# Mattdl/CLsurvey

Measured on AMD Instinct MI355X. Metric: images/sec (train+importance pass), EWC small_VGG9 Tiny-ImageNet task batch, higher is better.
Workload: dtype f32 (bf16x6 split operands on the conv fwd/bwd-data matrix products, fp32 accumulate); 1 GPU; EWC small_VGG9_cl_128_128, Tiny-ImageNet shapes (3x64x64, 20 classes), batch 200: train step + Fisher step (BASELINE configs[1]); batch=200, parallelism=1 GPU

## Files before the change

### clsurvey_amd/_lib.py

```python
import ctypes as C
import os

_HERE = os.path.dirname(os.path.abspath(__file__))
LIB_PATH = os.path.join(_HERE, "libclhip.so")

_p = C.c_void_p
_i = C.c_int
_f = C.c_float
_z = C.c_size_t
_l = C.c_long


class HatParam(C.Structure):
    _fields_ = [("theta", _p), ("grad", _p), ("buf", _p), ("mask_back", _p), ("n", _z), ("is_emb", _i), ("reserved", _i)]


class HatGateJob(C.Structure):
    _fields_ = [("emb_row", _p), ("gate", _p), ("mask_pre", _p), ("n", _i), ("reserved", _i)]


class HatLayer(C.Structure):
    _fields_ = [("w", _p), ("gate_in", _p), ("out", _p), ("K", _z), ("C", _z), ("R", _z)]


class HatWgradJob(C.Structure):
    _fields_ = [("g", _p), ("w", _p), ("gate_in", _p), ("dgate_in", _p), ("K", _i), ("C", _i), ("R", _i), ("reserved", _i)]


class HatEmbJob(C.Structure):
    _fields_ = [("dgate", _p), ("gate", _p), ("mask_pre", _p), ("demb", _p), ("n", _i), ("rows", _i), ("t", _i), ("reserved", _i)]


class PathnetLayer(C.Structure):
    _fields_ = [("w_off", _l), ("b_off", _l), ("pw_off", _l), ("pb_off", _l), ("mod_stride", _l), ("c_out", _i), ("c_in", _i),
                ("R", _i), ("n_out", _i), ("n_in", _i), ("Kp", _i), ("Cp", _i), ("M", _i), ("path", _i * 8),
                ("trainable", C.c_ulonglong)]


class IcarlClass(C.Structure):
    _fields_ = [("row_begin", _i), ("row_end", _i), ("k", _i), ("out_off", _i)]


class ReduceJob(C.Structure):
    _fields_ = [("slabs", _p), ("dw", _p), ("db", _p), ("K", _i), ("C", _i), ("splits", _i), ("taps", _i)]


class LayerDesc(C.Structure):
    _fields_ = [("type", _i), ("cin", _i), ("cout", _i), ("relu", _i), ("pool", _i),
                ("w_off", _l), ("b_off", _l), ("ksize", _i), ("stride", _i), ("pad", _i), ("pool_k", _i), ("pool_s", _i),
                ("bn", _i), ("bn_w_off", _l), ("bn_b_off", _l), ("has_drop", _i)]


SIGNATURES = {
    "clhip_version": (_i, []),
    "clhip_arch": (C.c_char_p, []),
    "clhip_conv3x3_fwd": (_i, [_p, _p, _p, _p, _i, _i, _i, _i, _i, _i, _p]),
    "clhip_conv3x3_relu_pool_fwd": (_i, [_p, _p, _p, _p, _p, _i, _i, _i, _i, _i, _p]),
    "clhip_conv3x3_bwd_weight_unpool": (_i, [_p, _p, _p, _p, _p, _i, _i, _i, _i, _i, _p, _z, _p]),
    "clhip_conv3x3_bwd_data": (_i, [_p, _p, _p, _p, _i, _i, _i, _i, _i, _p]),
    "clhip_conv3x3_bwd_data_unpool": (_i, [_p, _p, _p, _p, _p, _i, _i, _i, _i, _i, _p]),
    "clhip_conv3x3_bwd_weight_ws": (_z, [_i, _i, _i, _i, _i]),
    "clhip_conv3x3_bwd_weight": (_i, [_p, _p, _p, _p, _i, _i, _i, _i, _i, _p, _z, _p]),
    "clhip_conv3x3_bwd_weight_slabs": (_i, [_p, _p, _p, _i, _i, _i, _i, _i, _p, _z, C.POINTER(_i), _p]),
    "clhip_conv3x3_bwd_weight_reduce": (_i, [_p, _p, _p, _i, _i, _i, _p]),
    "clhip_conv3x3_wino_ws": (_z, [_i, _i]),
    "clhip_conv3x3_wino_fwd": (_i, [_p, _p, _p, _p, _p, _i, _i, _i, _i, _i, _i, _p, _z, _p]),
    "clhip_conv3x3_wino_bwd_data": (_i, [_p, _p, _p, _p, _p, _i, _i, _i, _i, _i, _p, _z, _p]),
    "clhip_conv5x5_bs_ws": (_z, [_i, _i]),
    "clhip_conv5x5_bs_fwd": (_i, [_p, _p, _p, _p, _i, _i, _i, _i, _i, _i, _p, _z, _p]),
    "clhip_conv5x5_bs_bwd_data": (_i, [_p, _p, _p, _p, _i, _i, _i, _i, _i, _p, _z, _p]),
    "clhip_conv3x3_bs_ws": (_z, [_i, _i]),
    "clhip_conv3x3_bs_fwd": (_i, [_p, _p, _p, _p, _p, _i, _i, _i, _i, _i, _i, _p, _z, _p]),
    "clhip_conv3x3_bs_bwd_data": (_i, [_p, _p, _p, _p, _p, _i, _i, _i, _i, _i, _p, _z, _p]),
    "clhip_conv3x3_bs_bwd_data_riders": (_i, [_p, _p, _p, _p, _p, _i, _i, _i, _i, _i, _p, _z, C.POINTER(ReduceJob), _i, _i, _i, _p]),
    "clhip_conv3x3_wino_bwd_weight_ws": (_z, [_i, _i, _i, _i, _i]),
    "clhip_conv3x3_wino_bwd_weight": (_i, [_p, _p, _p, _p, _p, _i, _i, _i, _i, _i, _p, _z, _p]),
    "clhip_conv3x3_wino_bwd_ws": (_z, [_i, _i, _i, _i, _i]),
    "clhip_conv3x3_wino_bwd": (_i, [_p, _p, _p, _p, _p, _p, _p, _p, _i, _i, _i, _i, _i, _p, _z, _p]),
    "clhip_maxpool2_fwd": (_i, [_p, _p, _p, _i, _i, _i, _p]),
    "clhip_maxpool2_bwd": (_i, [_p, _p, _p, _i, _i, _i, _p]),
    "clhip_fc_ws": (_z, [_i, _i, _i]),
    "clhip_fc_fwd": (_i, [_p, _p, _p, _p, _i, _i, _i, _i, _p, _z, _p]),
    "clhip_fc_bwd_data": (_i, [_p, _p, _p, _p, _i, _i, _i, _p, _z, _p]),
    "clhip_fc_bwd_weight": (_i, [_p, _p, _p, _p, _i, _i, _i, _p, _z, _p]),
    "clhip_relu_bwd": (_i, [_p, _p, _p, _z, _p]),
    "clhip_softmax_ce": (_i, [_p, _p, _i, _i, _i, _p, _p, _p, _p]),
    "clhip_mse_zero_sum": (_i, [_p, _z, _p, _p, _p]),
    "clhip_reg_sgd_step": (_i, [_p, _p, _p, _p, _p, _z, _f, _f, _f, _f, _i, _p]),
    "clhip_fisher_accum": (_i, [_p, _p, _z, _f, _p]),
    "clhip_mas_accum": (_i, [_p, _p, _z, _f, _f, _p]),
    "clhip_si_step": (_i, [_p, _p, _p, _p, _p, _p, _z, _f, _f, _f, _f, _i, _p]),
    "clhip_si_consolidate": (_i, [_p, _p, _p, _p, _z, _f, _p]),
    "clhip_maxpool_fwd": (_i, [_p, _p, _p, _i, _i, _i, _i, _i, _p]),
    "clhip_maxpool_bwd": (_i, [_p, _p, _p, _i, _i, _i, _i, _i, _p]),
    "clhip_conv2d_bwd_weight_ws": (_z, [_i] * 9),
    "clhip_conv2d_fwd": (_i, [_p, _p, _p, _p] + [_i] * 10 + [_p]),
    "clhip_conv2d_bwd_data": (_i, [_p, _p, _p, _p] + [_i] * 9 + [_p]),
    "clhip_conv2d_bwd_weight": (_i, [_p, _p, _p, _p] + [_i] * 9 + [_p, _z, _p]),
    "clhip_conv3x3_bs_bwd_weight_ws": (_z, [_i] * 5),
    "clhip_conv3x3_bs_bwd_weight": (_i, [_p] * 5 + [_i] * 5 + [_p, _z, _p]),
    "clhip_conv5x5_bs_bwd_weight_ws": (_z, [_i] * 5),
    "clhip_conv5x5_bs_bwd_weight": (_i, [_p] * 4 + [_i] * 5 + [_p, _z, _p]),
    "clhip_conv2d_s2d_ws": (_z, [_i] * 8),
    "clhip_conv2d_s2d_fwd": (_i, [_p, _p, _p, _p] + [_i] * 9 + [_p, _z, _p]),
    "clhip_conv2d_s2d_bwd_weight": (_i, [_p, _p, _p, _p] + [_i] * 8 + [_p, _z, _p]),
    "clhip_imm_merge": (_i, [_p, _p, _p, _i, _z, _p, _p]),
    "clhip_lwf_loss": (_i, [_p, _p, _p, _p, _i, _i, _i, _i, _f, _f, _i, _p, _p, _p, _p]),
    "clhip_packnet_finetune_mask": (_i, [_p, _z, _i, _p]),
    "clhip_packnet_kth_ws": (_z, []),
    "clhip_packnet_kth_abs": (_i, [_p, _p, _z, _i, _z, _p, _p, _z, _p]),
    "clhip_packnet_prune": (_i, [_p, _p, _z, _i, _p, _p]),
    "clhip_mask_grad_zero": (_i, [_p, _p, _z, _i, _p]),
    "clhip_mask_weight_zero": (_i, [_p, _p, _z, _i, _i, _p]),
    "clhip_packnet_sgd_step": (_i, [_p, _p, _p, _p, _z, _i, _f, _f, _f, _i, _p]),
    "clhip_hat_gate": (_i, [_p, _i, _f, _p, _p]),
    "clhip_hat_scale_weight": (_i, [_p, _p, _p, _z, _z, _z, _p]),
    "clhip_hat_weight_grad": (_i, [_p, _p, _p, _p, _p, _i, _i, _i, _p]),
    "clhip_hat_emb_grad": (_i, [_p, _p, _p, _i, _f, _f, _p, _p]),
    "clhip_hat_reg_sums": (_i, [_p, _p, _i, _p, _p]),
    "clhip_hat_backmask": (_i, [_p, _p, _p, _z, _z, _z, _p]),
    "clhip_hat_sgd_ws": (_z, []),
    "clhip_hat_sgd_step": (_i, [_p, _p, _p, _p, _z, _f, _f, _f, _i, _i, _f, _f, _f, _f, _i, _p, _z, _p]),
    "clhip_clamp": (_i, [_p, _z, _f, _f, _p]),
    "clhip_hat_sgd_multi_ws": (_z, [_i]),
    "clhip_hat_sgd_step_multi": (_i, [_p, _i, _f, _f, _f, _i, _f, _f, _f, _f, _f, _i, _p, _z, _p]),
    "clhip_hat_gates_multi": (_i, [_p, _i, _f, _p, _p]),
    "clhip_hat_scale_weights_multi": (_i, [_p, _i, _p]),
    "clhip_hat_weight_grads_multi": (_i, [_p, _i, _p]),
    "clhip_hat_emb_grads_multi": (_i, [_p, _i, _f, _f, _f, _p, _p]),
    "clhip_pathnet_ws": (_z, [_p, _i]),
    "clhip_pathnet_pack_multi": (_i, [_p, _i, _p, _z, _p, _z, _p]),
    "clhip_pathnet_fold_grads_multi": (_i, [_p, _i, _p, _z, _p, _z, _p, _z, _p]),
    "clhip_pathnet_sgd_step": (_i, [_p, _i, _p, _p, _p, _z, _f, _f, _f, _f, _i, _p, _z, _p]),
    "clhip_softmax_ce_slice": (_i, [_p, _p, _i, _i, _i, _i, _i, _p, _p, _p, _p]),
    "clhip_net_loss_step_slice": (_i, [_p, _p, _p, _p, _p, _i, _i, _i, _i, _p, _p, _p, _p, _p]),
    "clhip_axpy": (_i, [_p, _p, _z, _f, _i, _p]),
    "clhip_gem_gram_ws": (_z, [_i]),
    "clhip_gem_gram": (_i, [_p, _z, C.POINTER(_i), _i, _z, _p, _p, _z, _p]),
    "clhip_gem_project": (_i, [_p, _z, C.POINTER(_i), C.POINTER(_f), _i, _p, _p, _z, _p]),
    "clhip_gem_qp": (_i, [_p, _i, C.c_double, C.c_double, _p, _p, _p]),
# ... 101 lines not shown
```

### clsurvey_amd/build.py

```python
import glob
import os
import subprocess
import sys

HERE = os.path.dirname(os.path.abspath(__file__))
CSRC = os.path.join(HERE, "csrc")
OUT = os.path.join(HERE, "libclhip.so")
SOURCES = ["elementwise.hip", "loss.hip", "pool.hip", "conv3x3.hip", "wino.hip", "bsconv.hip", "bswgrad.hip", "bswgrad5.hip", "conv3x3_wgrad.hip", "conv2d.hip", "convkk.hip", "s2dconv.hip", "bn.hip", "gemm.hip", "fc_chain.hip",
           "packnet.hip", "hat.hip", "pathnet.hip", "gem.hip", "gem_wide.hip", "rehearsal.hip", "joint.hip", "augment.hip", "icarl.hip", "icarl_assemble.hip", "engine.hip"]
FLAGS = ["--offload-arch=gfx950", "-O3", "-std=c++17", "-fPIC", "-fvisibility=hidden", "-Wall", "-Wno-unused-function",
         "-mllvm", "-pragma-unroll-threshold=100000"]


EXTRA_FLAGS = {"wino.hip": ["-fno-slp-vectorize"]}


def _fingerprint(paths, flags):
    import hashlib
    h = hashlib.sha256(" ".join(flags).encode())
    for path in paths:
        with open(path, "rb") as f:
            h.update(f.read())
    return h.hexdigest()


def build(force=False, verbose=True):
    hipcc = os.environ.get("HIPCC", "/opt/rocm/bin/hipcc")
    objs = []
    hdrs = sorted(glob.glob(os.path.join(CSRC, "*.hpp"))) + [os.path.join(HERE, "..", "include", "clhip.h")]
    procs = []
    for src in SOURCES:
        s = os.path.join(CSRC, src)
        o = os.path.join(CSRC, src.replace(".hip", ".o"))
        stamp = o + ".sha256"
        objs.append(o)
        flags = FLAGS + EXTRA_FLAGS.get(src, [])
        want = _fingerprint([s] + hdrs, flags)
        have = open(stamp).read().strip() if os.path.exists(stamp) and os.path.exists(o) else ""
        if force or have != want:
            cmd = [hipcc] + flags + ["-c", s, "-o", o]
            if verbose:
                print(" ".join(cmd), flush=True)
            if os.path.exists(stamp):
                os.remove(stamp)
            procs.append((src, stamp, want, subprocess.Popen(cmd)))
    for src, stamp, want, p in procs:
        if p.wait() != 0:
            raise RuntimeError("hipcc failed on " + src)
        with open(stamp, "w") as f:
            f.write(want + "\n")
    if force or procs or not os.path.exists(OUT):
        cmd = [hipcc, "--offload-arch=gfx950", "-shared", "-fPIC", "-o", OUT] + objs
        if verbose:
            print(" ".join(cmd), flush=True)
        subprocess.check_call(cmd)
    return OUT


TEST_LIB_SRC = os.path.join(HERE, "..", "tests", "csrc", "debug_naive.hip")
TEST_LIB = os.path.join(HERE, "..", "tests", "libclhip_dbg.so")


def build_test_lib(force=False, verbose=True):
    hipcc = os.environ.get("HIPCC", "/opt/rocm/bin/hipcc")
    stamp = TEST_LIB + ".sha256"
    want = _fingerprint([TEST_LIB_SRC, os.path.join(CSRC, "common.hpp"), os.path.join(HERE, "..", "include", "clhip.h")], FLAGS)
    have = open(stamp).read().strip() if os.path.exists(stamp) and os.path.exists(TEST_LIB) else ""
    if force or have != want:
        cmd = [hipcc] + FLAGS + ["-shared", "-o", TEST_LIB, TEST_LIB_SRC]
        if verbose:
            print(" ".join(cmd), flush=True)
        subprocess.check_call(cmd)
        with open(stamp, "w") as f:
            f.write(want + "\n")
    return TEST_LIB


def build_variant(name, src, defines, verbose=True, extra_flags=()):
    hipcc = os.environ.get("HIPCC", "/opt/rocm/bin/hipcc")
    build(verbose=verbose)
    srcs = [src] if isinstance(src, str) else list(src)
    procs = []
    for s in srcs:
        o = os.path.join(CSRC, s.replace(".hip", ".%s.o" % name))
        cmd = [hipcc] + FLAGS + EXTRA_FLAGS.get(s, []) + list(extra_flags) + ["-D" + d for d in defines] + ["-c", os.path.join(CSRC, s), "-o", o]
        if verbose:
            print(" ".join(cmd), flush=True)
        procs.append(subprocess.Popen(cmd))
    for p in procs:
        if p.wait() != 0:
            raise RuntimeError("hipcc failed on variant " + name)
    objs = [os.path.join(CSRC, x.replace(".hip", ".%s.o" % name if x in srcs else ".o")) for x in SOURCES]
    out = os.path.join(HERE, "libclhip_%s.so" % name)
    subprocess.check_call([hipcc, "--offload-arch=gfx950", "-shared", "-fPIC", "-o", out] + objs)
    return out


# ... 4 lines not shown
```

### clsurvey_amd/csrc/common.hpp

```cpp
#pragma once
#include <hip/hip_runtime.h>
#include <stdint.h>
#include <stddef.h>
#include "../../include/clhip.h"

#define CLHIP_LAUNCH_CHECK()                          \
    do {                                              \
        hipError_t e__ = hipGetLastError();           \
        if (e__ != hipSuccess) return (int)e__;       \
    } while (0)

static inline hipStream_t as_stream(void* s) { return reinterpret_cast<hipStream_t>(s); }

static inline bool aligned16(const void* p) { return (reinterpret_cast<uintptr_t>(p) & 15u) == 0; }

static inline bool clhip_conv3x3_dims_ok(int N, int C, int K, int H, int W) {
    if (N <= 0 || C <= 0 || K <= 0 || H <= 0 || W <= 0) return false;
    const long long hw = (long long)H * W;
    if (hw >= (1LL << 23)) return false;
    if (hw * (C + 32LL) >= (1LL << 28) || hw * (K + 32LL) >= (1LL << 28)) return false;
    if ((long long)K * C >= (1LL << 29) / 9) return false;
    return hw * N <= 0x7fffffffLL;
}

// ... 45 lines not shown
    __builtin_amdgcn_raw_buffer_store_b128(q, r, voff, soff, CLHIP_ST_AUX);
}
__device__ __forceinline__ void clhip_buf_store2(float2 v, __amdgpu_buffer_rsrc_t r, int voff, int soff) {
    typedef unsigned int u32x2 __attribute__((ext_vector_type(2)));
    const u32x2 q = {__float_as_uint(v.x), __float_as_uint(v.y)};
    __builtin_amdgcn_raw_buffer_store_b64(q, r, voff, soff, CLHIP_ST_AUX);
}
__device__ __forceinline__ __amdgpu_buffer_rsrc_t clhip_out_rsrc(void* base) {
    return __builtin_amdgcn_make_buffer_rsrc(base, 0, 0x7fffffff, 0x00020000);
}
__device__ __forceinline__ size_t out_img_of(int C, int hw) { return (size_t)C * hw; }

__device__ __forceinline__ float wave_max(float v) {
#pragma unroll
    for (int o = 32; o > 0; o >>= 1) v = fmaxf(v, __shfl_xor(v, o, 64));
    return v;
}
__device__ __forceinline__ float wave_sum(float v) {
#pragma unroll
    for (int o = 32; o > 0; o >>= 1) v += __shfl_xor(v, o, 64);
    return v;
}
__device__ __forceinline__ double wave_sum(double v) {
#pragma unroll
    for (int o = 32; o > 0; o >>= 1) v += __shfl_xor(v, o, 64);
    return v;
}
__device__ __forceinline__ int wave_min(int v) {
#pragma unroll
    for (int o = 32; o > 0; o >>= 1) v = min(v, __shfl_xor(v, o, 64));
    return v;
}

typedef float floatx16 __attribute__((ext_vector_type(16)));
typedef float floatx4 __attribute__((ext_vector_type(4)));

__device__ __forceinline__ int mfma32_row(int r, int lane) { return (r & 3) + 8 * (r >> 2) + 4 * (lane >> 5); }


#define CLHIP_FC_MAX 4
struct clhip_fc_chain {
    int n;
    long w_off[CLHIP_FC_MAX], b_off[CLHIP_FC_MAX];
    int din[CLHIP_FC_MAX], dout[CLHIP_FC_MAX], relu[CLHIP_FC_MAX];
    size_t act_off[CLHIP_FC_MAX], dz_off[CLHIP_FC_MAX];
};
int clhip_internal_fc_chain_ok(const clhip_fc_chain* d);
int clhip_internal_fc_chain_wgrad(const clhip_fc_chain* d, float* grads, const float* x, int N, const float* acts,
                                  const float* dlogits, const float* dz, hipStream_t s);
struct clhip_gemm_args {
    const float* a; const float* b; float* out;
    int M, N, K; long sam, sak, sbk, sbn; int n_tiles, splits, k_per_split;
    const float* bias; const float* mask_src; int relu;
};
int clhip_internal_fc_bwd_data_args(const float* dy, const float* w, const float* relu_src, float* dx, int M, int I, int O,
                                    clhip_gemm_args* args_out);
int clhip_internal_fc_bwd_combo(const clhip_gemm_args* g, int gemm_blocks, const clhip_fc_chain* d, float* grads, const float* x,
                                int N, const float* acts, const float* dlogits, const float* dz, hipStream_t s);

int clhip_internal_fc_tail_ok(const clhip_fc_chain* d);
int clhip_internal_fc_tail(const clhip_fc_chain* d, const float* params, float* acts, int N, const int64_t* labels,
                           int reduction, int col_off, int ncols, float* dlogits, float* fcdz, float* loss_out, double* stats,
                           void* row_scratch, unsigned* counter, int do_loss, int do_bwd, const float* h1_slabs, int live,
                           hipStream_t s);
int clhip_internal_fc_fwd_partial(const float* x, const float* w, int M, int I, int O, void* ws, size_t ws_bytes, int* live,
                                  hipStream_t s);

#define CLHIP_WGRAD_JOBS_MAX 32
struct clhip_wgrad_job { const float* part; float* dw; float* db; int K, C, splits; int taps; };
int clhip_internal_conv3x3_wgrad_partial(const float* x, const float* dy, const uint8_t* unpool_idx, float* dw, float* db, int N,
                                         int C, int K, int H, int W, void* ws, size_t ws_bytes, void* stream, clhip_wgrad_job* job);
int clhip_internal_wgrad_reduce_multi(const clhip_wgrad_job* jobs, int n, hipStream_t s);

bool clhip_internal_convkk_ok(int N, int Cin, int Cout, int H, int W, int R, int S, int stride, int pad);
int clhip_internal_convkk(int mode, const float* in, const float* w, const float* bias, const float* mask_src, float* out, int N,
                          int Cin, int Cout, int H, int W, int relu, hipStream_t s);

struct clhip_wino_wt { const float* w; float* U; int Ko, Ci, mode, pad; };
int clhip_internal_wino_weights(const clhip_wino_wt* jobs, int n, hipStream_t s);
int clhip_internal_weight_images(const clhip_wino_wt* wino_jobs, int n_wino, const clhip_wino_wt* bs_jobs, int n_bs, hipStream_t s);
int clhip_internal_c3w64_pool_weight_images(const float* x, const float* w, const float* b, float* y_pool, uint8_t* idx_u8, int N, int C,
                                            int K, int H, int W, const clhip_wino_wt* wino_jobs, int n_wino, const clhip_wino_wt* bs_jobs,
                                            int n_bs, int wt_first, hipStream_t s);
int clhip_internal_wino_conv_u(int mode, const float* in, const float* U, const float* bias, const float* mask_src, float* out,
                               uint8_t* pool_idx, int unpool, int N, int Cin, int Cout, int H, int W, int relu, hipStream_t s);
bool clhip_internal_wino_ok(int Cin, int Cout, int H, int W);
size_t clhip_internal_wino_ws(int Cin, int Cout);
bool clhip_internal_bs_ok(int Cin, int Cout, int H, int W);
bool clhip_internal_bs_index_ok(int Cin, int Cout, int H, int W, int ks);
bool clhip_internal_bs_preferred(int Cin, int Cout, int H, int W);
bool clhip_internal_bs5_preferred(int Cin, int Cout, int H, int W);
size_t clhip_internal_bs5_ws(int Cin, int Cout);
int clhip_internal_bs5_conv_u(int mode, const float* in, const void* wimg, const float* bias, const float* mask_src, float* out, int N,
                              int Cin, int Cout, int H, int W, int relu, hipStream_t s);
size_t clhip_internal_bs_ws(int Cin, int Cout);
int clhip_internal_bs_weights(const clhip_wino_wt* jobs, int n, hipStream_t s);
int clhip_internal_bs_conv_u(int mode, const float* in, const void* wimg, const float* bias, const float* mask_src, float* out,
                             uint8_t* pool_idx, int unpool, int N, int Cin, int Cout, int H, int W, int relu, hipStream_t s);
int clhip_internal_bs_conv_u_riders(const float* in, const void* wimg, const float* mask_src, float* out, uint8_t* pool_idx, int unpool,
                                    int N, int Cin, int Cout, int H, int W, const clhip_wgrad_job* jobs, int n_jobs, int place,
                                    int riders, hipStream_t s);
bool clhip_internal_bs5_wgrad_ok(int N, int C, int K, int H, int W);
size_t clhip_internal_bs5_wgrad_ws(int N, int C, int K, int H, int W);
int clhip_internal_bs5_wgrad(const float* x, const float* dy, float* dw, float* db, int N, int C, int K, int H, int W, void* ws,
                             size_t ws_bytes, hipStream_t s);
size_t clhip_internal_bs3k_wgrad_ws(int N, int C, int K, int H, int W);
int clhip_internal_bs3k_wgrad(const float* x, const float* dy, float* dw, float* db, int N, int C, int K, int H, int W, void* ws,
                              size_t ws_bytes, hipStream_t s);
bool clhip_internal_bs_wgrad_ok(int C, int K, int H, int W);
bool clhip_internal_bs_wgrad_preferred(int C, int K, int H, int W, int pooled);
size_t clhip_internal_bs_wgrad_ws(int N, int C, int K, int H, int W);
int clhip_internal_bs_wgrad_partial(const float* x, const float* dy, const uint8_t* unpool_idx, float* dw, float* db, int N, int C, int K,
                                    int H, int W, void* ws, size_t ws_bytes, hipStream_t s, clhip_wgrad_job* job);
bool clhip_internal_wino_wgrad_ok(int C, int K, int H, int W);
size_t clhip_internal_wino_wgrad_ws(int N, int C, int K, int H, int W);
int clhip_internal_wino_wgrad_partial(const float* x, const float* dy, const uint8_t* unpool_idx, float* dw, float* db, int N, int C,
                                      int K, int H, int W, void* ws, size_t ws_bytes, hipStream_t s, clhip_wgrad_job* job);
int clhip_internal_wino_pair(const float* dy, const uint8_t* unpool_idx, const float* U, const float* mask_src, float* dx,
                             const float* x, float* dw, float* db, int N, int C, int K, int H, int W, void* ws, size_t ws_bytes,
                             hipStream_t s, clhip_wgrad_job* job);
bool clhip_internal_wino_pair_shape(int N, int C, int K, int H, int W, int pooled);
int clhip_internal_wino_conv(int mode, const float* in, const float* w, const float* bias, const float* mask_src, float* out,
                             uint8_t* pool_idx, int unpool, int N, int Cin, int Cout, int H, int W, int relu, void* ws,
                             size_t ws_bytes, hipStream_t s);
```

### clsurvey_amd/csrc/conv3x3.hip

```cpp
#include "common.hpp"
#include "weight_images.hpp"

namespace {

#ifdef CLHIP_TRACE
__device__ unsigned long long* g_trace = nullptr;
#define TR_NOW() __builtin_amdgcn_s_memtime()
#endif

constexpr int KT = 64;
constexpr int LDW = 65;

template <int TW, int TH, int NB>
struct Geo {
    static constexpr int BP = TW * TH * NB;
    static constexpr int TWP = TW + 2;
    static constexpr int PLANE = NB * (TH + 2) * TWP;
    static constexpr int NT = (BP + 63) / 64;
    static constexpr bool DENSE = (32 % TW != 0 && TW != 32);
    static_assert(DENSE || BP == 64 || BP == 128, "block tile must hold 64 or 128 pixels");
    static_assert(!DENSE || (NB == 1 && BP <= 192), "dense tiles: one plane of at most 192 pixels");
};

template <int TW, int TH>
// ... 960 lines not shown

int launch_c3w64_pool_wt(const float* x, const float* wt, const float* bias, float* out, uint8_t* idx, int N, int Cout, int H, int W,
                         const WtJobs& J, int wt_first, hipStream_t s) {
    const int tiles_w = W / 64, row_pairs = H / 2;
    const long long ntiles = (long long)tiles_w * row_pairs * N;
    const int kts = (Cout + KT - 1) / KT;
    const long long gx = c3w64_gx(ntiles);
    const int nfl = (int)(gx * kts), nwb = (J.first[J.n] + 1) / 2;
    if (Cout % KT == 0)
        hipLaunchKernelGGL(c3w64_relu_pool_wt_kernel<true>, dim3((unsigned)(nfl + nwb)), dim3(512), 0, s,
                           x, wt, bias, out, idx, N, Cout, H, W, tiles_w, row_pairs, (int)ntiles, (int)gx, nfl, nwb, wt_first, J);
    else
        hipLaunchKernelGGL(c3w64_relu_pool_wt_kernel<false>, dim3((unsigned)(nfl + nwb)), dim3(512), 0, s,
                           x, wt, bias, out, idx, N, Cout, H, W, tiles_w, row_pairs, (int)ntiles, (int)gx, nfl, nwb, wt_first, J);
    CLHIP_LAUNCH_CHECK();
    return 0;
}

int launch_c3w64_pool(const float* x, const float* wt, const float* bias, float* out, uint8_t* idx,
                      int N, int Cout, int H, int W, hipStream_t s) {
    const int tiles_w = W / 64, row_pairs = H / 2;
    const long long ntiles = (long long)tiles_w * row_pairs * N;
    const int kts = (Cout + KT - 1) / KT;
    const long long gx = c3w64_gx(ntiles);
    if (Cout % KT == 0)
        hipLaunchKernelGGL(conv3x3_c3w64_relu_pool_kernel<true>, dim3((unsigned)gx, (unsigned)kts), dim3(512), 0, s,
                           x, wt, bias, out, idx, N, Cout, H, W, tiles_w, row_pairs, (int)ntiles);
    else
        hipLaunchKernelGGL(conv3x3_c3w64_relu_pool_kernel<false>, dim3((unsigned)gx, (unsigned)kts), dim3(512), 0, s,
                           x, wt, bias, out, idx, N, Cout, H, W, tiles_w, row_pairs, (int)ntiles);
    CLHIP_LAUNCH_CHECK();
    return 0;
}

int launch_c3_pool(const float* x, const float* wt, const float* bias, float* out, uint8_t* idx,
                   int N, int Cout, int H, int W, hipStream_t s) {
    const int tiles_w = W / C3_TW, tiles_h = (H + C3_TH - 1) / C3_TH;
    const long long ntiles = (long long)tiles_w * tiles_h * N;
    const int kts = (Cout + KT - 1) / KT;
    if (ntiles <= 0 || ntiles > 0x7fffffffLL) return CLHIP_EINVAL;
    long long gx = 512 / kts;
    if (gx < 1) gx = 1;
    if (gx > ntiles) gx = ntiles;
    hipLaunchKernelGGL(conv3x3_c3_relu_pool_kernel, dim3((unsigned)gx, (unsigned)kts), dim3(256), 0, s,
                       x, wt, bias, out, idx, N, Cout, H, W, tiles_w, tiles_h, (int)ntiles);
    CLHIP_LAUNCH_CHECK();
    return 0;
}

bool c3w64_shape(int N, int C, int K, int H, int W) {
    return C == 3 && W % 64 == 0 && H % 2 == 0 && (size_t)N * 3 * H * W < ((size_t)1 << 29) &&
           (size_t)N * K * (H / 2) * (W / 2) < ((size_t)1 << 29);
}

bool vec_ok(const float* in, const float* wt, int Cin, int H, int W, int Cw) {
    const int TW = W > 16 ? 32 : (W > 8 ? 16 : 8);
    return (Cin % 8 == 0) && (Cw % 4 == 0) && (W % 4 == 0) && (W % TW == 0) && aligned16(in) && aligned16(wt);
}

}

extern "C" {

#ifdef CLHIP_TRACE
int clhip_debug_set_conv_trace(void* p) {
    unsigned long long* q = static_cast<unsigned long long*>(p);
    return (int)hipMemcpyToSymbol(HIP_SYMBOL(g_trace), &q, sizeof(q));
}
#endif

int clhip_conv3x3_fwd(const float* x, const float* w, const float* b, float* y,
                      int N, int C, int K, int H, int W, int relu, void* stream) {
    if (!x || !w || !y || !clhip_conv3x3_dims_ok(N, C, K, H, W)) return CLHIP_EINVAL;
    hipStream_t s = as_stream(stream);
    if (C <= 4) return launch_conv<4, 0, false>(x, w, b, nullptr, y, N, C, K, H, W, K, C, relu, s);
    if (vec_ok(x, w, C, H, W, C)) return launch_conv<8, 0, true>(x, w, b, nullptr, y, N, C, K, H, W, K, C, relu, s);
    return launch_conv<8, 0, false>(x, w, b, nullptr, y, N, C, K, H, W, K, C, relu, s);
}

int clhip_conv3x3_relu_pool_fwd(const float* x, const float* w, const float* b, float* y_pool, uint8_t* idx_u8,
                                int N, int C, int K, int H, int W, void* stream) {
    if (!x || !w || !y_pool || !idx_u8 || !clhip_conv3x3_dims_ok(N, C, K, H, W) || (H & 1) || (W & 1)) return CLHIP_EINVAL;
    hipStream_t s = as_stream(stream);
    if (c3w64_shape(N, C, K, H, W)) return launch_c3w64_pool(x, w, b, y_pool, idx_u8, N, K, H, W, s);
    if (C == 3 && W % C3_TW == 0 && aligned16(y_pool) && aligned16(idx_u8)) return launch_c3_pool(x, w, b, y_pool, idx_u8, N, K, H, W, s);

    if (C <= 4) return launch_conv<4, 0, false>(x, w, b, nullptr, y_pool, N, C, K, H, W, K, C, 1, s, idx_u8);
    if (vec_ok(x, w, C, H, W, C)) return launch_conv<8, 0, true>(x, w, b, nullptr, y_pool, N, C, K, H, W, K, C, 1, s, idx_u8);
    return launch_conv<8, 0, false>(x, w, b, nullptr, y_pool, N, C, K, H, W, K, C, 1, s, idx_u8);
}

}

int clhip_internal_c3w64_pool_weight_images(const float* x, const float* w, const float* b, float* y_pool, uint8_t* idx_u8, int N, int C,
                                            int K, int H, int W, const clhip_wino_wt* wj, int nw, const clhip_wino_wt* bj, int nb,
                                            int wt_first, hipStream_t s) {
    if (!x || !w || !y_pool || !idx_u8 || N <= 0 || C <= 0 || K <= 0 || H <= 0 || W <= 0) return CLHIP_EINVAL;
    if (!c3w64_shape(N, C, K, H, W) || nw < 0 || nb < 0 || nw + nb <= 0 || nw + nb > WT_JOBS) return CLHIP_ENOTSUP;
    WtJobs J;
    const int blocks = weight_jobs_table(wj, nw, bj, nb, J);
    if (blocks < 0) return blocks;
    return launch_c3w64_pool_wt(x, w, b, y_pool, idx_u8, N, K, H, W, J, wt_first, s);
}

extern "C" {

int clhip_conv3x3_bwd_data(const float* dy, const float* w, const float* relu_src, float* dx,
                           int N, int C, int K, int H, int W, void* stream) {
    if (!dy || !w || !dx || !clhip_conv3x3_dims_ok(N, C, K, H, W)) return CLHIP_EINVAL;
    if (vec_ok(dy, w, K, H, W, C))
        return launch_conv<8, 1, true>(dy, w, nullptr, relu_src, dx, N, K, C, H, W, K, C, 0, as_stream(stream));
    return launch_conv<8, 1, false>(dy, w, nullptr, relu_src, dx, N, K, C, H, W, K, C, 0, as_stream(stream));
}

int clhip_conv3x3_bwd_data_unpool(const float* dy_pool, const uint8_t* idx_u8, const float* w, const float* relu_src, float* dx,
                                  int N, int C, int K, int H, int W, void* stream) {
    if (!dy_pool || !idx_u8 || !w || !dx || !clhip_conv3x3_dims_ok(N, C, K, H, W)) return CLHIP_EINVAL;
    if ((H & 1) || (W & 1) || !vec_ok(dy_pool, w, K, H, W, C) || (reinterpret_cast<uintptr_t>(idx_u8) & 1u)) return CLHIP_ENOTSUP;
    return launch_conv<8, 1, true, true>(dy_pool, w, nullptr, relu_src, dx, N, K, C, H, W, K, C, 0, as_stream(stream),
                                         const_cast<uint8_t*>(idx_u8));
}

}
```

### include/clhip.h

```cpp
#ifndef CLHIP_H
#define CLHIP_H

#include <stddef.h>
#include <stdint.h>

#ifdef __cplusplus
extern "C" {
#endif

#if defined(__GNUC__) || defined(__clang__)
#pragma GCC visibility push(default)
#define CLHIP_VISIBILITY_PUSHED 1
#endif

#define CLHIP_EINVAL (-1)
#define CLHIP_ENOSPC (-2)
#define CLHIP_ENOTSUP (-3)

int clhip_sigmoid_fwd(const float* x, float* y, size_t n, void* stream);
int clhip_sigmoid_bwd(const float* dy, const float* y, float* dx, size_t n, void* stream);
int clhip_mse_mean(const float* a, const float* b, size_t n, float grad_scale, float* da, float* loss_out, void* stream);
int clhip_adadelta_step(float* theta, const float* grad, float* square_avg, float* acc_delta, size_t n, float lr, float rho,
                        float eps, float weight_decay, void* stream);

int clhip_version(void);
const char* clhip_arch(void);

int clhip_conv3x3_fwd(const float* x, const float* w, const float* b, float* y,
                      int N, int C, int K, int H, int W, int relu, void* stream);

int clhip_conv3x3_relu_pool_fwd(const float* x, const float* w, const float* b, float* y_pool, uint8_t* idx_u8,
                                int N, int C, int K, int H, int W, void* stream);

int clhip_conv3x3_bwd_data(const float* dy, const float* w, const float* relu_src, float* dx,
                           int N, int C, int K, int H, int W, void* stream);

size_t clhip_conv3x3_bwd_weight_ws(int N, int C, int K, int H, int W);
int clhip_conv3x3_bwd_weight(const float* x, const float* dy, float* dw, float* db,
                             int N, int C, int K, int H, int W, void* ws, size_t ws_bytes,
                             void* stream);

int clhip_conv3x3_bwd_data_unpool(const float* dy_pool, const uint8_t* idx_u8, const float* w, const float* relu_src,
                                  float* dx, int N, int C, int K, int H, int W, void* stream);

int clhip_conv3x3_bwd_weight_slabs(const float* x, const float* dy, const uint8_t* idx_u8_or_null, int N, int C, int K,
                                   int H, int W, void* ws, size_t ws_bytes, int* splits_out, void* stream);
int clhip_conv3x3_bwd_weight_reduce(const void* ws, float* dw, float* db, int K, int C, int splits, void* stream);

int clhip_conv3x3_bwd_weight_unpool(const float* x, const float* dy_pool, const uint8_t* idx_u8, float* dw, float* db,
                                    int N, int C, int K, int H, int W, void* ws, size_t ws_bytes, void* stream);

int clhip_maxpool2_fwd(const float* x, float* y, uint8_t* idx_u8, int NC, int H, int W, void* stream);
int clhip_maxpool2_bwd(const float* dy, const uint8_t* idx_u8, float* dx, int NC, int H, int W,
                       void* stream);

int clhip_maxpool_fwd(const float* x, float* y, uint8_t* idx_u8, int NC, int H, int W, int k, int stride, void* stream);
int clhip_maxpool_bwd(const float* dy, const uint8_t* idx_u8, float* dx, int NC, int H, int W, int k, int stride, void* stream);

size_t clhip_bn_ws(int C);
int clhip_bn_fwd(const float* z, const float* gamma, const float* beta, float* running_mean, float* running_var, float* y,
                 float* save_mean, float* save_invstd, int N, int C, int HW, int training, float momentum, float eps, int relu,
                 void* ws, size_t ws_bytes, void* stream);
int clhip_bn_bwd(const float* dy, const float* y, const float* z, const float* gamma, const float* save_mean,
                 const float* save_invstd, float* dz, float* dgamma, float* dbeta, int N, int C, int HW, int training, int relu,
                 void* ws, size_t ws_bytes, void* stream);

size_t clhip_conv2d_bwd_weight_ws(int N, int C, int H, int W, int K, int R, int S, int stride, int pad);
int clhip_conv2d_fwd(const float* x, const float* w, const float* b, float* y, int N, int C, int H, int W, int K, int R, int S,
                     int stride, int pad, int relu, void* stream);
int clhip_conv2d_bwd_data(const float* dy, const float* w, const float* relu_src, float* dx, int N, int C, int H, int W, int K,
                          int R, int S, int stride, int pad, void* stream);
int clhip_conv2d_bwd_weight(const float* x, const float* dy, float* dw, float* db, int N, int C, int H, int W, int K, int R,
                            int S, int stride, int pad, void* ws, size_t ws_bytes, void* stream);

size_t clhip_conv3x3_bs_bwd_weight_ws(int N, int C, int K, int H, int W);
int clhip_conv3x3_bs_bwd_weight(const float* x, const float* dy, const uint8_t* idx_u8_or_null, float* dw, float* db, int N, int C, int K,
                                int H, int W, void* ws, size_t ws_bytes, void* stream);

size_t clhip_conv5x5_bs_bwd_weight_ws(int N, int C, int K, int H, int W);
int clhip_conv5x5_bs_bwd_weight(const float* x, const float* dy, float* dw, float* db, int N, int C, int K, int H, int W, void* ws,
                                size_t ws_bytes, void* stream);

size_t clhip_conv2d_s2d_ws(int N, int C, int H, int W, int K, int R, int stride, int pad);
int clhip_conv2d_s2d_fwd(const float* x, const float* w, const float* b, float* y, int N, int C, int H, int W, int K, int R, int stride,
                         int pad, int relu, void* ws, size_t ws_bytes, void* stream);
int clhip_conv2d_s2d_bwd_weight(const float* x_or_null, const float* dy, float* dw, float* db, int N, int C, int H, int W, int K, int R,
                                int stride, int pad, void* ws, size_t ws_bytes, void* stream);

size_t clhip_fc_ws(int M, int I, int O);
int clhip_fc_fwd(const float* x, const float* w, const float* b, float* y,
                 int M, int I, int O, int relu, void* ws, size_t ws_bytes, void* stream);
int clhip_fc_bwd_data(const float* dy, const float* w, const float* relu_src, float* dx,
                      int M, int I, int O, void* ws, size_t ws_bytes, void* stream);
int clhip_fc_bwd_weight(const float* x, const float* dy, float* dw, float* db,
                        int M, int I, int O, void* ws, size_t ws_bytes, void* stream);
int clhip_relu_bwd(const float* dy, const float* y, float* dx, size_t n, void* stream);

int clhip_softmax_ce(const float* logits, const int64_t* labels_i64, int N, int C, int reduction,
                     float* dlogits, float* loss_out, double* stats, void* stream);
int clhip_softmax_ce_slice(const float* logits, const int64_t* labels_i64, int N, int ld, int col_off, int ncols,
                           int reduction, float* dlogits, float* loss_out, double* stats, void* stream);
int clhip_mse_zero_sum(const float* logits, size_t n, float* dlogits, float* loss_out, void* stream);

int clhip_lwf_loss(const float* logits, const int64_t* labels_i64, const float* teacher, const int* head_sizes, int n_heads,
                   int N, int ld, int ld_teacher, float T, float reg_lambda, int distill, float* dlogits, float* loss_out2,
                   double* stats, void* stream);

int clhip_reg_sgd_step(float* theta, const float* grad, const float* omega, const float* init_val,
                       float* buf, size_t n, float reg_lambda, float lr, float momentum, float wd,
                       int first, void* stream);
int clhip_fisher_accum(float* omega, const float* grad, size_t n, float data_len, void* stream);
int clhip_mas_accum(float* omega, const float* grad, size_t n, float prev_size, float curr_size,
                    void* stream);
int clhip_si_step(float* theta, const float* grad, const float* omega, const float* init_val,
                  float* w, float* buf, size_t n, float reg_lambda, float lr, float momentum,
// ... 296 lines not shown
```

Before: 303,300 images/s.

## Add MFMA bf16x3-split first-layer conv+relu+pool kernel for 3-channel input

Adds a new kernel for the first 3-input-channel 3x3 conv with fused ReLU and 2x2 max-pool. It packs the 27 taps into bf16 MFMA 32x32x16 operands using a three-way bf16 split for near-fp32 accuracy, with double-buffered LDS input tiles and a persistent-style split of tiles across SIMDs. It also has a variant that co-schedules weight-image preparation blocks. It is enabled by default through an environment switch and replaces the previous scalar/vector c3w64 path. The cost is more split-product MFMA work and some zero padding in the K dimension.

```diff
diff --git a/clsurvey_amd/_lib.py b/clsurvey_amd/_lib.py
--- a/clsurvey_amd/_lib.py
+++ b/clsurvey_amd/_lib.py
@@ -56,6 +56,7 @@
     "clhip_arch": (C.c_char_p, []),
     "clhip_conv3x3_fwd": (_i, [_p, _p, _p, _p, _i, _i, _i, _i, _i, _i, _p]),
     "clhip_conv3x3_relu_pool_fwd": (_i, [_p, _p, _p, _p, _p, _i, _i, _i, _i, _i, _p]),
+    "clhip_conv3x3_c3_path": (_i, []),
     "clhip_conv3x3_bwd_weight_unpool": (_i, [_p, _p, _p, _p, _p, _i, _i, _i, _i, _i, _p, _z, _p]),
     "clhip_conv3x3_bwd_data": (_i, [_p, _p, _p, _p, _i, _i, _i, _i, _i, _p]),
     "clhip_conv3x3_bwd_data_unpool": (_i, [_p, _p, _p, _p, _p, _i, _i, _i, _i, _i, _p]),
diff --git a/clsurvey_amd/build.py b/clsurvey_amd/build.py
--- a/clsurvey_amd/build.py
+++ b/clsurvey_amd/build.py
@@ -6,13 +6,13 @@
 HERE = os.path.dirname(os.path.abspath(__file__))
 CSRC = os.path.join(HERE, "csrc")
 OUT = os.path.join(HERE, "libclhip.so")
-SOURCES = ["elementwise.hip", "loss.hip", "pool.hip", "conv3x3.hip", "wino.hip", "bsconv.hip", "bswgrad.hip", "bswgrad5.hip", "conv3x3_wgrad.hip", "conv2d.hip", "convkk.hip", "s2dconv.hip", "bn.hip", "gemm.hip", "fc_chain.hip",
+SOURCES = ["elementwise.hip", "loss.hip", "pool.hip", "conv3x3.hip", "c3bs.hip", "wino.hip", "bsconv.hip", "bswgrad.hip", "bswgrad5.hip", "conv3x3_wgrad.hip", "conv2d.hip", "convkk.hip", "s2dconv.hip", "bn.hip", "gemm.hip", "fc_chain.hip",
            "packnet.hip", "hat.hip", "pathnet.hip", "gem.hip", "gem_wide.hip", "rehearsal.hip", "joint.hip", "augment.hip", "icarl.hip", "icarl_assemble.hip", "engine.hip"]
 FLAGS = ["--offload-arch=gfx950", "-O3", "-std=c++17", "-fPIC", "-fvisibility=hidden", "-Wall", "-Wno-unused-function",
          "-mllvm", "-pragma-unroll-threshold=100000"]
 
 
-EXTRA_FLAGS = {"wino.hip": ["-fno-slp-vectorize"]}
+EXTRA_FLAGS = {"wino.hip": ["-fno-slp-vectorize"], "c3bs.hip": ["-fno-slp-vectorize"]}
 
 
 def _fingerprint(paths, flags):
diff --git a/clsurvey_amd/csrc/c3bs.hip b/clsurvey_amd/csrc/c3bs.hip
--- /dev/null
+++ b/clsurvey_amd/csrc/c3bs.hip
@@ -0,0 +1,330 @@
+#include "common.hpp"
+#include "weight_images.hpp"
+#include <cstdlib>
+
+#ifndef C3BS_ABL
+#define C3BS_ABL 0
+#endif
+
+namespace {
+
+constexpr int B3_KT = 64;
+constexpr int B3_RS = 33;
+constexpr int B3_PIECE = 12 * B3_RS;
+constexpr int B3_BUF = 3 * B3_PIECE;
+constexpr int B3_LDS = 8 * 2 * B3_BUF;
+constexpr int B3_WIMG = 2 * 2 * 3 * 64;
+
+__device__ __forceinline__ bool b3_slot(int st, int kk, int e, int& c, int& r, int& s) {
+    c = 0; r = 0; s = 0;
+    if (e < 6) {
+        s = e % 3;
+        const int second = e / 3;
+        if (st == 0) { c = kk; r = second; }
+        else if (kk == 0) { c = 2; r = second; }
+        else { c = second; r = 2; }
+        return true;
+    }
+    if (st == 1) return false;
+    c = 2; r = 2;
+    if (kk == 0) { s = e - 6; return true; }
+    s = 2;
+    return e == 7;
+}
+
+__device__ __forceinline__ unsigned b3_align16(unsigned hi, unsigned lo) { return (lo >> 16) | (hi << 16); }
+
+typedef unsigned int b3_u32x2 __attribute__((ext_vector_type(2)));
+__device__ __forceinline__ void b3_operands(b3_u32x2 a, b3_u32x2 b, unsigned last0, unsigned last1, clhip_u32x4& p0, clhip_u32x4& p1) {
+    p0 = clhip_u32x4{a.x, (a.y & 0xffffu) | (b.x << 16), b3_align16(b.y, b.x), last0};
+    p1 = clhip_u32x4{b3_align16(a.y, a.x), (a.y >> 16) | (b.x & 0xffff0000u), b.y, last1};
+}
+
+template <bool FULL>
+__device__ __forceinline__ void c3bs_relu_pool_body(
+    unsigned* __restrict__ lds, clhip_u32x4* __restrict__ wimg, float* __restrict__ bias_s, const int bx, const int by, const int gx,
+    const float* __restrict__ x, const float* __restrict__ wt, const float* __restrict__ bias,
+    float* __restrict__ out, uint8_t* __restrict__ pool_idx, int N, int Cout, int H, int W,
+    int tiles_w, int row_pairs, int ntiles) {
+    const int tid = threadIdx.x, lane = tid & 63, wave = tid >> 6, li = lane & 31, kk = lane >> 5;
+    const int ko0 = by * B3_KT;
+    if (tid < B3_KT) bias_s[tid] = (bias && ko0 + tid < Cout) ? bias[ko0 + tid] : 0.f;
+
+    if (wave < 4) {
+        const int half = wave >> 1, st = wave & 1;
+        const int ch = ko0 + 32 * half + li;
+        float v[8];
+#pragma unroll
+        for (int e = 0; e < 8; ++e) {
+            int c0, r0, s0, c1, r1, s1;
+            const bool real0 = b3_slot(0, 0, e, c0, r0, s0), real1 = b3_slot(0, 1, e, c1, r1, s1);
+            int c2, r2, s2, c3, r3, s3;
+            const bool real2 = b3_slot(1, 0, e, c2, r2, s2), real3 = b3_slot(1, 1, e, c3, r3, s3);
+            const bool real = st ? (kk ? real3 : real2) : (kk ? real1 : real0);
+            const int t = st ? (kk ? c3 * 9 + r3 * 3 + s3 : c2 * 9 + r2 * 3 + s2) : (kk ? c1 * 9 + r1 * 3 + s1 : c0 * 9 + r0 * 3 + s0);
+            v[e] = (real && ch < Cout) ? wt[(size_t)ch * 27 + t] : 0.f;
+        }
+        clhip_u32x4 q[3];
+        bs_split8(v, q[0], q[1], q[2]);
+#pragma unroll
+        for (int pc = 0; pc < 3; ++pc) wimg[(wave * 3 + pc) * 64 + lane] = q[pc];
+    }
+    const clhip_u32x4* const wl = wimg + lane;
+
+    const int o_s0 = li + kk * 4 * B3_RS;
+    const int o_g = li + (2 * 4 + 2) * B3_RS;
+    const int o_s1 = li + (kk ? 2 : 8) * B3_RS;
+    const int d_s1 = (kk ? 4 : 1) * B3_RS;
+
+    const int simd = bx * 4 + (wave & 3), nsimd = gx * 4;
+    const int units = 2 * ntiles;
+    const int per = units / nsimd, rem = units - per * nsimd;
+    const int s_start = simd * per + min(simd, rem), s_cnt = per + (simd < rem ? 1 : 0);
+    const int first = (s_cnt + 1) >> 1;
+    const int u0 = __builtin_amdgcn_readfirstlane((wave >> 2) ? s_start + first : s_start);
+    const int u1 = __builtin_amdgcn_readfirstlane((wave >> 2) ? s_start + s_cnt : s_start + first);
+
+    const size_t plane_hw = (size_t)H * W;
+    const __amdgpu_buffer_rsrc_t r_x = clhip_rsrc(x, (size_t)N * 3 * plane_hw * 4);
+    float sv[13];
+    const int e_line = lane >> 1, e_side = lane & 1, e_c = e_line >> 2, e_rr = e_line & 3;
+    auto tile_coords = [&](int t, int& n, int& h, int& w0) {
+        const int tw = t % tiles_w, q = t / tiles_w;
+        const int rp = q % row_pairs;
+        n = q / row_pairs; h = 2 * rp; w0 = tw * 64;
+    };
+    auto load_tile = [&](int t) {
+        int n, h, w0;
+        tile_coords(t, n, h, w0);
+        const int base = (n * 3 * H + h - 1) * W + w0;
+#pragma unroll
+        for (int i = 0; i < 12; ++i) {
+            const int c = i >> 2, rr = i & 3;
+            const bool ok = (unsigned)(h - 1 + rr) < (unsigned)H;
+            sv[i] = clhip_buf_load(r_x, ok ? (base + (c * H + rr) * W + lane) * 4 : CLHIP_OOB, 0);
+        }
+        const int ecol = w0 + (e_side ? 64 : -1);
+        const bool eok = (lane < 24) & ((unsigned)(h - 1 + e_rr) < (unsigned)H) & ((unsigned)ecol < (unsigned)W);
+        sv[12] = clhip_buf_load(r_x, eok ? ((n * 3 * H + h - 1) * W + (e_c * H + e_rr) * W + ecol) * 4 : CLHIP_OOB, 0);
+    };
+    unsigned* hw_s = lds + wave * (2 * B3_BUF);
+    auto store_tile = [&](int buf) {
+        unsigned short* d = reinterpret_cast<unsigned short*>(hw_s + buf * B3_BUF);
+#pragma unroll
+        for (int i = 0; i < 6; ++i) {
+            unsigned p[3];
+            bs_split2(sv[2 * i], sv[2 * i + 1], p[0], p[1], p[2]);
+#pragma unroll
+            for (int pc = 0; pc < 3; ++pc) {
+                d[2 * (pc * B3_PIECE + (2 * i) * B3_RS) + 1 + lane] = (unsigned short)(p[pc] & 0xffffu);
+                d[2 * (pc * B3_PIECE + (2 * i + 1) * B3_RS) + 1 + lane] = (unsigned short)(p[pc] >> 16);
+            }
+        }
+        unsigned p[3];
+        bs_split2(sv[12], 0.f, p[0], p[1], p[2]);
+        if (lane < 24) {
+#pragma unroll
+            for (int pc = 0; pc < 3; ++pc) d[2 * (pc * B3_PIECE + e_line * B3_RS) + (e_side ? 65 : 0)] = (unsigned short)(p[pc] & 0xffffu);
+        }
+    };
+
+    const int OH = H >> 1, OW = W >> 1;
+    const int chw = OH * OW;
+    const __amdgpu_buffer_rsrc_t r_o = clhip_rsrc(out, (size_t)N * Cout * chw * 4);
+    const __amdgpu_buffer_rsrc_t r_i = clhip_rsrc(pool_idx, (size_t)N * Cout * chw);
+    __syncthreads();
+    if (u0 >= u1) return;
+
+    floatx16 acc[2][2], accl[2][2];
+    int buf = 0;
+
+    auto compute = [&](const int half) {
+        const unsigned* xs = hw_s + buf * B3_BUF;
+#pragma unroll
+        for (int st = 0; st < 2; ++st) {
+            clhip_u32x4 xq[2][2][3];
+            clhip_u32x4 wh[3];
+#pragma unroll
+            for (int pc = 0; pc < 3; ++pc) wh[pc] = wl[((2 * half + st) * 3 + pc) * 64];
+#if C3BS_ABL & 2
+#pragma unroll
+            for (int row = 0; row < 2; ++row)
+#pragma unroll
+                for (int par = 0; par < 2; ++par)
+#pragma unroll
+                    for (int pc = 0; pc < 3; ++pc)
+                        xq[row][par][pc] = clhip_u32x4{(unsigned)lane, (unsigned)(row * 2 + par), (unsigned)st, (unsigned)pc};
+#else
+#pragma unroll
+            for (int pc = 0; pc < 3; ++pc) {
+                const unsigned* xp = xs + pc * B3_PIECE;
+                if (st == 0) {
+                    b3_u32x2 ln[3], g[2];
+#pragma unroll
+                    for (int hr = 0; hr < 3; ++hr) ln[hr] = b3_u32x2{xp[o_s0 + hr * B3_RS], xp[o_s0 + hr * B3_RS + 1]};
+#pragma unroll
+                    for (int row = 0; row < 2; ++row) g[row] = b3_u32x2{xp[o_g + row * B3_RS], xp[o_g + row * B3_RS + 1]};
+#pragma unroll
+                    for (int row = 0; row < 2; ++row) {
+                        const unsigned mid = b3_align16(g[row].y, g[row].x);
+                        b3_operands(ln[row], ln[row + 1], kk ? mid : g[row].x, kk ? g[row].y : mid, xq[row][0][pc], xq[row][1][pc]);
+                    }
+                } else {
+#pragma unroll
+                    for (int row = 0; row < 2; ++row) {
+                        const int oa = o_s1 + row * B3_RS, ob = oa + d_s1;
+                        b3_operands(b3_u32x2{xp[oa], xp[oa + 1]}, b3_u32x2{xp[ob], xp[ob + 1]}, 0u, 0u, xq[row][0][pc], xq[row][1][pc]);
+                    }
+                }
+            }
+#endif
+#if C3BS_ABL & 1
+#define C3BS_TERM(ACC, PX, PW, FIRST)                                                                                              \
+            _Pragma("unroll") for (int row = 0; row < 2; ++row) _Pragma("unroll") for (int par = 0; par < 2; ++par) {              \
+                if (FIRST) ACC[row][par] = floatx16{0.f, 0.f, 0.f, 0.f, 0.f, 0.f, 0.f, 0.f, 0.f, 0.f, 0.f, 0.f, 0.f, 0.f, 0.f, 0.f}; \
+                asm volatile("" : "+v"(ACC[row][par]) : "v"(xq[row][par][PX]), "v"(wh[PW]));                                   \
+            }
+#else
+#define C3BS_TERM(ACC, PX, PW, FIRST)                                                                                              \
+            _Pragma("unroll") for (int row = 0; row < 2; ++row) _Pragma("unroll") for (int par = 0; par < 2; ++par) {              \
+                const floatx16 zero = {0.f, 0.f, 0.f, 0.f, 0.f, 0.f, 0.f, 0.f, 0.f, 0.f, 0.f, 0.f, 0.f, 0.f, 0.f, 0.f};            \
+                ACC[row][par] = __builtin_amdgcn_mfma_f32_32x32x16_bf16(__builtin_bit_cast(bs_bf16x8, wh[PW]),                 \
+                                                                       __builtin_bit_cast(bs_bf16x8, xq[row][par][PX]),           \
+                                                                       (FIRST) ? zero : ACC[row][par], 0, 0, 0);                   \
+            }
+#endif
+            C3BS_TERM(accl, 0, 2, st == 0) C3BS_TERM(acc, 0, 0, st == 0) C3BS_TERM(accl, 2, 0, false) C3BS_TERM(accl, 1, 1, false)
+            C3BS_TERM(accl, 0, 1, false) C3BS_TERM(accl, 1, 0, false)
+#undef C3BS_TERM
+        }
+    };
+
+    int t_cur = u0 >> 1;
+    const int t_last = (u1 - 1) >> 1;
+    load_tile(t_cur);
+    store_tile(0);
+    if (t_cur < t_last) load_tile(t_cur + 1);
+    for (int u = u0; u < u1; ++u) {
+        const int t = u >> 1, half = u & 1;
+        compute(half);
+        const bool last_of_tile = u + 1 < u1 && ((u + 1) >> 1) != t;
+        if (last_of_tile) {
+            store_tile(buf ^ 1);
+            t_cur = t + 1;
+            if (t_cur < t_last) load_tile(t_cur + 1);
+        }
+        int n, h, w0;
+        tile_coords(t, n, h, w0);
+        const int cbase = ko0 + 32 * half;
+        const int obase = ((n * Cout + cbase) * OH + (h >> 1)) * OW + (w0 >> 1);
+        const int ovoff = (4 * kk * chw + li);
+#pragma unroll
+        for (int r = 0; r < 16; ++r) {
+            const int c0 = (r & 3) + 8 * (r >> 2);
+            const float bv = bias_s[32 * half + 4 * kk + c0];
+            const float tl = (acc[0][0][r] + accl[0][0][r]) + bv, tr = (acc[0][1][r] + accl[0][1][r]) + bv;
+            const float bl = (acc[1][0][r] + accl[1][0][r]) + bv, br = (acc[1][1][r] + accl[1][1][r]) + bv;
+            float mx, m;
+            asm("v_max3_f32 %0, %1, %2, %3" : "=v"(mx) : "v"(tl), "v"(tr), "v"(bl));
+            asm("v_max_f32 %0, %1, %2" : "=v"(mx) : "v"(mx), "v"(br));
+            int am = 3;
+            am = bl == mx ? 2 : am;
+            am = tr == mx ? 1 : am;
+            am = tl == mx ? 0 : am;
+            if (!(mx > 0.f)) am = CLHIP_POOL_DEAD;
+            asm("v_max_f32 %0, 0, %1" : "=v"(m) : "v"(mx));
+            m = (__builtin_isunordered(tl, tr) | __builtin_isunordered(bl, br)) ? __builtin_nanf("") : m;
+            const bool cok = (FULL || cbase + c0 + 4 * kk < Cout) && !(C3BS_ABL & 4);
+            clhip_buf_store(m, r_o, cok ? ovoff * 4 : CLHIP_OOB, (obase + c0 * chw) * 4);
+            clhip_buf_store_u8((uint8_t)am, r_i, cok ? ovoff : CLHIP_OOB, obase + c0 * chw);
+        }
+        if (last_of_tile) buf ^= 1;
+    }
+}
+
+template <bool FULL>
+__global__ __launch_bounds__(512) void c3bs_relu_pool_kernel(
+    const float* __restrict__ x, const float* __restrict__ wt, const float* __restrict__ bias,
+    float* __restrict__ out, uint8_t* __restrict__ pool_idx, int N, int Cout, int H, int W,
+    int tiles_w, int row_pairs, int ntiles) {
+    __shared__ __attribute__((aligned(16))) unsigned lds[B3_LDS];
+    __shared__ clhip_u32x4 wimg[B3_WIMG];
+    __shared__ float bias_s[B3_KT];
+    c3bs_relu_pool_body<FULL>(lds, wimg, bias_s, (int)blockIdx.x, (int)blockIdx.y, (int)gridDim.x, x, wt, bias, out, pool_idx, N, Cout, H, W,
+                              tiles_w, row_pairs, ntiles);
+}
+
+template <bool FULL>
+__global__ __launch_bounds__(512) void c3bs_relu_pool_wt_kernel(
+    const float* __restrict__ x, const float* __restrict__ wt, const float* __restrict__ bias,
+    float* __restrict__ out, uint8_t* __restrict__ pool_idx, int N, int Cout, int H, int W,
+    int tiles_w, int row_pairs, int ntiles, int gx, int nfl, int nwb, int wt_first, WtJobs J) {
+    __shared__ __attribute__((aligned(16))) unsigned lds[B3_LDS];
+    __shared__ clhip_u32x4 wimg[B3_WIMG];
+    __shared__ float bias_s[B3_KT];
+    const int b = (int)blockIdx.x;
+    const int fb = wt_first ? b - nwb : b;
+    if ((unsigned)fb >= (unsigned)nfl) {
+        const int vb = 2 * (wt_first ? b : b - nfl) + ((int)threadIdx.x >> 8);
+        if (vb < J.first[J.n]) weight_image_block(J, vb, (int)threadIdx.x & 255);
+        return;
+    }
+    c3bs_relu_pool_body<FULL>(lds, wimg, bias_s, fb % gx, fb / gx, gx, x, wt, bias, out, pool_idx, N, Cout, H, W, tiles_w, row_pairs, ntiles);
+}
+
+static inline long long c3bs_gx(long long ntiles) {
+    long long gx = 256;
+    if (gx * 8 > 2 * ntiles) gx = (2 * ntiles + 7) / 8;
+    return gx;
+}
+
+int g_c3_path = -1;
+
+}
+
+#ifndef CLHIP_C3_BS_DEFAULT
+#define CLHIP_C3_BS_DEFAULT 1
+#endif
+int clhip_internal_c3_bs_mode() {
+    const char* e = std::getenv("CLHIP_C3_BS");
+    return (e && (e[0] == '0' || e[0] == '1') && !e[1]) ? e[0] - '0' : CLHIP_C3_BS_DEFAULT;
+}
+void clhip_internal_c3_path_note(int body) { g_c3_path = body; }
+
+int clhip_internal_c3bs_pool(const float* x, const float* wt, const float* bias, float* out, uint8_t* idx, int N, int Cout, int H, int W,
+                             hipStream_t s) {
+    const int tiles_w = W / 64, row_pairs = H / 2;
+    const long long ntiles = (long long)tiles_w * row_pairs * N;
+    const int kts = (Cout + B3_KT - 1) / B3_KT;
+    const long long gx = c3bs_gx(ntiles);
+    if (Cout % B3_KT == 0)
+        hipLaunchKernelGGL(c3bs_relu_pool_kernel<true>, dim3((unsigned)gx, (unsigned)kts), dim3(512), 0, s,
+                           x, wt, bias, out, idx, N, Cout, H, W, tiles_w, row_pairs, (int)ntiles);
+    else
+        hipLaunchKernelGGL(c3bs_relu_pool_kernel<false>, dim3((unsigned)gx, (unsigned)kts), dim3(512), 0, s,
+                           x, wt, bias, out, idx, N, Cout, H, W, tiles_w, row_pairs, (int)ntiles);
+    CLHIP_LAUNCH_CHECK();
+    return 0;
+}
+
+int clhip_internal_c3bs_pool_wt(const float* x, const float* wt, const float* bias, float* out, uint8_t* idx, int N, int Cout, int H, int W,
+                                const clhip_wino_wt* wj, int nw, const clhip_wino_wt* bj, int nb, int wt_first, hipStream_t s) {
+    WtJobs J;
+    const int blocks = weight_jobs_table(wj, nw, bj, nb, J);
+    if (blocks < 0) return blocks;
+    const int tiles_w = W / 64, row_pairs = H / 2;
+    const long long ntiles = (long long)tiles_w * row_pairs * N;
+    const int kts = (Cout + B3_KT - 1) / B3_KT;
+    const long long gx = c3bs_gx(ntiles);
+    const int nfl = (int)(gx * kts), nwb = (J.first[J.n] + 1) / 2;
+    if (Cout % B3_KT == 0)
+        hipLaunchKernelGGL(c3bs_relu_pool_wt_kernel<true>, dim3((unsigned)(nfl + nwb)), dim3(512), 0, s,
+                           x, wt, bias, out, idx, N, Cout, H, W, tiles_w, row_pairs, (int)ntiles, (int)gx, nfl, nwb, wt_first, J);
+    else
+        hipLaunchKernelGGL(c3bs_relu_pool_wt_kernel<false>, dim3((unsigned)(nfl + nwb)), dim3(512), 0, s,
+                           x, wt, bias, out, idx, N, Cout, H, W, tiles_w, row_pairs, (int)ntiles, (int)gx, nfl, nwb, wt_first, J);
+    CLHIP_LAUNCH_CHECK();
+    return 0;
+}
+
+extern "C" int clhip_conv3x3_c3_path(void) { return g_c3_path; }
diff --git a/clsurvey_amd/csrc/common.hpp b/clsurvey_amd/csrc/common.hpp
--- a/clsurvey_amd/csrc/common.hpp
+++ b/clsurvey_amd/csrc/common.hpp
@@ -151,6 +151,13 @@
 int clhip_internal_c3w64_pool_weight_images(const float* x, const float* w, const float* b, float* y_pool, uint8_t* idx_u8, int N, int C,
                                             int K, int H, int W, const clhip_wino_wt* wino_jobs, int n_wino, const clhip_wino_wt* bs_jobs,
                                             int n_bs, int wt_first, hipStream_t s);
+int clhip_internal_c3_bs_mode();
+void clhip_internal_c3_path_note(int body);
+int clhip_internal_c3bs_pool(const float* x, const float* w, const float* b, float* y_pool, uint8_t* idx_u8, int N, int K, int H, int W,
+                             hipStream_t s);
+int clhip_internal_c3bs_pool_wt(const float* x, const float* w, const float* b, float* y_pool, uint8_t* idx_u8, int N, int K, int H, int W,
+                                const clhip_wino_wt* wino_jobs, int n_wino, const clhip_wino_wt* bs_jobs, int n_bs, int wt_first,
+                                hipStream_t s);
 int clhip_internal_wino_conv_u(int mode, const float* in, const float* U, const float* bias, const float* mask_src, float* out,
                                uint8_t* pool_idx, int unpool, int N, int Cin, int Cout, int H, int W, int relu, hipStream_t s);
 bool clhip_internal_wino_ok(int Cin, int Cout, int H, int W);
diff --git a/clsurvey_amd/csrc/conv3x3.hip b/clsurvey_amd/csrc/conv3x3.hip
--- a/clsurvey_amd/csrc/conv3x3.hip
+++ b/clsurvey_amd/csrc/conv3x3.hip
@@ -1066,7 +1066,11 @@
                                 int N, int C, int K, int H, int W, void* stream) {
     if (!x || !w || !y_pool || !idx_u8 || !clhip_conv3x3_dims_ok(N, C, K, H, W) || (H & 1) || (W & 1)) return CLHIP_EINVAL;
     hipStream_t s = as_stream(stream);
-    if (c3w64_shape(N, C, K, H, W)) return launch_c3w64_pool(x, w, b, y_pool, idx_u8, N, K, H, W, s);
+    if (c3w64_shape(N, C, K, H, W)) {
+        const int bs = clhip_internal_c3_bs_mode();
+        clhip_internal_c3_path_note(bs);
+        return bs ? clhip_internal_c3bs_pool(x, w, b, y_pool, idx_u8, N, K, H, W, s) : launch_c3w64_pool(x, w, b, y_pool, idx_u8, N, K, H, W, s);
+    }
     if (C == 3 && W % C3_TW == 0 && aligned16(y_pool) && aligned16(idx_u8)) return launch_c3_pool(x, w, b, y_pool, idx_u8, N, K, H, W, s);
 
     if (C <= 4) return launch_conv<4, 0, false>(x, w, b, nullptr, y_pool, N, C, K, H, W, K, C, 1, s, idx_u8);
@@ -1081,9 +1085,16 @@
                                             int wt_first, hipStream_t s) {
     if (!x || !w || !y_pool || !idx_u8 || N <= 0 || C <= 0 || K <= 0 || H <= 0 || W <= 0) return CLHIP_EINVAL;
     if (!c3w64_shape(N, C, K, H, W) || nw < 0 || nb < 0 || nw + nb <= 0 || nw + nb > WT_JOBS) return CLHIP_ENOTSUP;
+    const int bs = clhip_internal_c3_bs_mode();
+    if (bs) {
+        const int rc = clhip_internal_c3bs_pool_wt(x, w, b, y_pool, idx_u8, N, K, H, W, wj, nw, bj, nb, wt_first, s);
+        if (rc == 0) clhip_internal_c3_path_note(1);
+        return rc;
+    }
     WtJobs J;
     const int blocks = weight_jobs_table(wj, nw, bj, nb, J);
     if (blocks < 0) return blocks;
+    clhip_internal_c3_path_note(0);
     return launch_c3w64_pool_wt(x, w, b, y_pool, idx_u8, N, K, H, W, J, wt_first, s);
 }
 
diff --git a/include/clhip.h b/include/clhip.h
--- a/include/clhip.h
+++ b/include/clhip.h
@@ -31,6 +31,7 @@
 
 int clhip_conv3x3_relu_pool_fwd(const float* x, const float* w, const float* b, float* y_pool, uint8_t* idx_u8,
                                 int N, int C, int K, int H, int W, void* stream);
+int clhip_conv3x3_c3_path(void);
 
 int clhip_conv3x3_bwd_data(const float* dy, const float* w, const float* relu_src, float* dx,
                            int N, int C, int K, int H, int W, void* stream);
```

Result: no change. 306,100 images/s, median of 6 (+0.9%).
